# GloireLINVANI/3D_Gaussian_Splatting_Project

Measured on AMD Instinct MI355X. Metric: Gaussians·views/sec labelled (3M G, 1080p), majority vote; first vote_view submit -> labels on the host, higher is better.
Workload: dtype f64

## Files before the change

### 3d_gaussian_splatting_project_amd/csrc/gsx_ctx.hpp

```cpp
#pragma once
#include <hip/hip_runtime.h>

#include <chrono>
#include <cstdarg>
#include <cstdint>
#include <cstdio>
#include <map>
#include <cstddef>
#include <string>
#include <vector>

#include "../../include/gsx.h"
#include "host_pack.hpp"

namespace gsx {

void set_global_error(const char* fmt, ...);
struct Ctx;
int fail(Ctx* c, int code, const char* fmt, ...);

#define GSX_HIP(ctx, call)                                                                         \
    do {                                                                                           \
        hipError_t e__ = (call);                                                                   \
        if (e__ != hipSuccess)                                                                     \
// ... 224 lines not shown

    int64_t n = 0;
    int64_t n_pad = 0;
    DevBuf x, y, z;
    DevBuf perm;
    bool sorted = false;
    DevBuf sort_hist;

    int opt_spatial_sort = 1;
    int opt_xcd_swizzle = 32;
    int opt_vote_unroll = 8;
    int opt_slabs = 1;
    int opt_local_codes = 0;
    int opt_seg_tiled = 1;
    int opt_batched_counts = 1;
    int opt_seg_coarse = 1;
    int opt_flat_project = 1;

    bool vote_begun = false;
    int n_classes = 0, bins = 0;
    int first_view = 0, total_views = 0;
    bool wide = false;
    bool local_codes = false;
    int slabs = 1;
    int64_t sn = 0;
    std::vector<ViewDesc> views;
    DevBuf d_cull;
    int cull_pitch = 0;
    DevBuf d_cull_tally;
    int opt_wave_cull = 1;
    bool views_dirty = true;
    bool views_coarse = false;
    bool views_simple = false;
    DevBuf d_views;
    DevBuf segpool;
    size_t seg_used = 0;
    DevBuf errflag;
    HandOver ho;
    int opt_host_threads = 0;
    int opt_host_compact = 1;
#ifdef GSX_EXPERIMENTS
    int opt_ablate = 0;
#else
    static constexpr int opt_ablate = 0;
#endif
    int opt_labels_u8 = 1;
    int opt_host_pack = 1;
    void* h_labels = nullptr;
    size_t h_labels_cap = 0;
    hipEvent_t h_ev[kLabelChunks] = {nullptr, nullptr, nullptr, nullptr};
    void* h_views = nullptr;
    size_t h_views_cap = 0;
    hipEvent_t h_views_ev = nullptr;
    std::vector<ViewDesc> own_views;
    int own_first_view = 0;
    const void* pool_base = nullptr;
    int n_flushed = 0;
    bool planes_valid = false;
    bool planes_zero = false;
    bool planes_stale = false;
    DevBuf cnt, fv;
    DevBuf keys, labels;
    DevBuf labels8;
    DevBuf bcnt, bcodes;
    DevBuf cand, codes;
    long long counts_n = -1, counts_npad = -1, counts_sn = -1, codes_n = -1, codes_npad = -1;
    int counts_bins = -1;
    bool labels_valid = false;
    int opt_filter_project = 1;
    int opt_early_vote = 1;
    int opt_early_at = 0;
    std::chrono::steady_clock::time_point early_t0;
    int opt_early_replay = 1;
    bool early_replayed = false;
    int early_state = 0;
    int early_done = 0;
    int early_batches = 0;
    hipStream_t stream2 = nullptr;
    bool stream_borrowed = false;
    bool early_inflight = false;
    hipEvent_t early_maps_ev = nullptr, early_done_ev = nullptr, early_up_ev = nullptr;
    DevBuf ecnt, efv;
    DevBuf erec;
    DevBuf e_views, e_cull;
    void* h_early = nullptr;
    size_t h_early_cap = 0;

    RenderScene scene;
    RenderOpts ropt;
    RenderFrame frame;
    LiftState lift;
    Ctx* twins[kMaxFrames - 1] = {nullptr, nullptr, nullptr, nullptr, nullptr};
    DevBuf r_pre_args;
    std::vector<unsigned long long> r_pre_args_host;
    hipEvent_t r_pre_ev[kPreSets] = {nullptr, nullptr, nullptr};

    int opt_nn_brute = 0;
    DevBuf nn_index;
    int64_t nn_index_rows = 0;
    int nn_index_k = 0;
    DevBuf nn_pts, nn_cs;
    DevBuf nn_out, nn_flag;

    int opt_smooth_search = 0;
    DevBuf sm_lab[2];
    DevBuf sm_sup, sm_changed;
    DevBuf sm_lists;

    DevBuf sp_lab, sp_parent, sp_rep;
    DevBuf sp_size, sp_id, sp_kept;
    DevBuf sp_trip, sp_cnt;
    DevBuf sp_pts, sp_lists;

    int opt_iou_table_lds = 1;
    DevBuf iou_planes;
    DevBuf iou_cnt;
    DevBuf iou_ptrs;
    DevBuf iou_table;
    DevBuf iou_top;
    DevBuf iou_raw[2];
    void* iou_pin[2] = {nullptr, nullptr};
    size_t iou_pin_cap[2] = {0, 0};
    hipEvent_t iou_ev[2] = {nullptr, nullptr};
    bool iou_ev_pending[2] = {false, false};
    int iou_slot = 0;

    DevBuf seg_low;
    DevBuf q_bits;
    DevBuf q_parts;
    DevBuf q_tab;

    bool prof_on = false;
    std::vector<std::string> prof_names;
    std::vector<ProfEvent> prof_events;
    std::vector<hipEvent_t> event_pool;
    std::map<std::string, std::pair<int64_t, double>> prof_acc;
};

struct ProfScope {
    Ctx* c;
    ProfEvent ev{};
    bool active = false;
    hipStream_t st = nullptr;
    ProfScope(Ctx* ctx, const char* name, hipStream_t on = nullptr);
    ~ProfScope();
};

int vote_begin(Ctx* c, int n_classes, int first_view, int total_views);
int vote_view(Ctx* c, const gsx_camera* cam, const void* seg, int seg_dtype, int seg_w, int seg_h, int img_w, int img_h);
int early_pool_moves(Ctx* c);
void vote_release_host(Ctx* c);
int vote_slab_labels(Ctx* c, int slab, int slabs, int64_t* slab_size);
int vote_view_host(Ctx* c, const gsx_camera* cam, const void* seg, int seg_dtype, int seg_w, int seg_h, int img_w, int img_h);
int vote_views_device(Ctx* c, int n, const gsx_camera* cams, const void* const* segs, int seg_dtype, int seg_w, int seg_h,
                      int img_w, int img_h);
int vote_export(Ctx* c, int64_t reserve_bytes, void* blobs_out, void** pool_dev, int64_t* pool_bytes);
int vote_import(Ctx* c, int n_parts, const int32_t* part_views, const int64_t* part_offsets, const void* blobs,
                const void* pool_all_dev, int64_t pool_all_bytes);
int vote_import_uniform(Ctx* c, int n_parts, const int32_t* part_views, const int64_t* part_offsets, const gsx_camera* cams,
                        int seg_w, int seg_h, int img_w, int img_h, const void* pool_all_dev, int64_t pool_all_bytes);
int vote_import_undo(Ctx* c);
int vote_map_stride(Ctx* c, int seg_w, int seg_h, int64_t* stride);
int vote_views_match_uniform(Ctx* c, int n, const gsx_camera* cams, int seg_w, int seg_h, int img_w, int img_h, int32_t* match);
Workers* host_workers(Ctx* c, const void* near = nullptr);
int host_threads(Ctx* c);
int vote_flush_pending(Ctx* c);
void handover_release(Ctx* c);
// ... 124 lines not shown
```

### 3d_gaussian_splatting_project_amd/csrc/vote.hip

```cpp
#include <hip/hip_runtime.h>

#include <algorithm>
#include <chrono>
#include <cmath>
#include <cstring>
#include <type_traits>

#include "gsx_ctx.hpp"
#include "vote_device.hpp"

namespace gsx {

template <int DIV>
__global__ __launch_bounds__(kBlock) void project_kernel(const float* __restrict__ x, const float* __restrict__ y,
                                                         const float* __restrict__ z, long long n,
                                                         const ViewDesc* __restrict__ vd,
                                                         const uint32_t* __restrict__ perm, int* __restrict__ ox,
                                                         int* __restrict__ oy, float filt_h) {
    const long long i = (long long)blockIdx.x * kBlock + threadIdx.x;
    const bool valid = i < n;
    int xi, yi;
    const ViewRegs vr = load_view(vd);
    const double X = valid ? (double)x[i] : __builtin_nan(""), Y = valid ? (double)y[i] : 0.0, Z = valid ? (double)z[i] : 0.0;
    const bool vis = DIV == kDivFiltCoarse ? project_filtered(vr, filt_h, X, Y, Z, xi, yi) : project<DIV>(vr, X, Y, Z, xi, yi);
// ... 119 lines not shown
                                             double X, double Y, double Z, unsigned culled, int (&bin)[U], float filt_h) {
    if (DIV == kDivFlatCoarse || DIV == kDivFiltCoarse) {
        unsigned pixel[U];
#pragma unroll
        for (int u = 0; u < U; ++u) {
            const int v = vb - 1 - u;
            bin[u] = -1;
            if (((culled >> u) & 1u) || !(FULL || v >= 0)) continue;
            const ViewRegs vd = load_view(views + v);
            int xi, yi;
            if (DIV == kDivFiltCoarse ? project_filtered(vd, filt_h, X, Y, Z, xi, yi) : project<kDivFlatSimple>(vd, X, Y, Z, xi, yi)) {
                pixel[u] = (unsigned)xi | ((unsigned)yi << 16);
                const unsigned cx = (unsigned)xi >> 2, cy = (unsigned)yi >> 2;
                const unsigned coff = __umul24(cx >> 4, (unsigned)vd.coarse_row_bytes) + (cx & 15u) + (cy << 4);
                bin[u] = ((global_u8_ptr)((unsigned long long)vd.seg_off + vd.coarse_delta))[coff];
            }
        }
#pragma unroll
        for (int u = 0; u < U; ++u) {
            const bool mixed = bin[u] == 255;
            if (__builtin_amdgcn_ballot_w64(mixed) != 0) {
                const ViewDesc* __restrict__ vp = views + (vb - 1 - u);
                const global_u8_ptr base = (global_u8_ptr)(unsigned long long)vp->seg_off;
                const unsigned xi = pixel[u] & 0xffffu, yi = pixel[u] >> 16;
                if (mixed) bin[u] = base[__umul24(xi >> 4, (unsigned)vp->seg_row_bytes) + (xi & 15u) + (yi << 4)];
            }
        }
        return;
    }
#pragma unroll
    for (int u = 0; u < U; ++u) {
        const int v = vb - 1 - u;
        if ((culled >> u) & 1u) {
            bin[u] = -1;
            continue;
        }
        bin[u] = (FULL || v >= 0) ? seg_bin<DIV>(views + v, pool, X, Y, Z) : -1;
    }
}

template <int U, int DIV>
__global__ __launch_bounds__(kBlock) void vote_fused_labels_kernel(FusedParams p, const ViewDesc* __restrict__ views,
                                                                   int* __restrict__ labels) {
    extern __shared__ uint32_t lds[];
    uint32_t* row = lds + threadIdx.x * p.stride_dw;
    uint8_t* h = reinterpret_cast<uint8_t*>(row);

    for (int k = 0; k < p.stride_dw; ++k) row[k] = 0;
    const long long i = (long long)logical_block(blockIdx.x, gridDim.x, p.xcd_swizzle) * kBlock + threadIdx.x;
    const bool valid = i < p.n;
    const double X = valid ? (double)p.x[i] : __builtin_nan("");
    const double Y = valid ? (double)p.y[i] : 0.0;
    const double Z = valid ? (double)p.z[i] : 0.0;
    const uint8_t* __restrict__ pool = p.pool;

    int best = -1;
    int bestc = 0;
    const CullMasks cmask = wave_cull_masks(p.cull, p.cull_pitch, p.nviews, X, Y, Z, p.cull_tally);
    auto chunk = [&](auto full, int vb) {
        constexpr bool kFull = decltype(full)::value;
        int bin[U];
        gather_chunk<U, DIV, kFull>(views, pool, vb, X, Y, Z, cull_bits<U>(cmask, p.nviews - vb), bin, p.filt_h);
#pragma unroll
        for (int u = 0; u < U; ++u) {
            if (bin[u] >= 0) {
                const int c = h[bin[u]] + 1;
                h[bin[u]] = (uint8_t)c;
                if (c >= bestc) {
                    bestc = c;
                    best = bin[u];
                }
            }
        }
        };
    int vb = p.nviews;
    for (; vb >= U; vb -= U) chunk(std::true_type{}, vb);
    if (vb > 0) chunk(std::false_type{}, vb);
    if (valid) {
        const long long o = p.perm ? (long long)p.perm[i] : i;
        labels[o] = best - 1 + (best < 0);
    }
}

template <int U, int DIV>
__global__ __launch_bounds__(kBlock) void vote_record_kernel(FusedParams p, const ViewDesc* __restrict__ views,
                                                             uint8_t* __restrict__ rec) {
    const long long i = (long long)logical_block(blockIdx.x, gridDim.x, p.xcd_swizzle) * kBlock + threadIdx.x;
    const bool valid = i < p.n;
    const long long ic = valid ? i : 0;
    const float xf = p.x[ic], yf = p.y[ic], zf = p.z[ic];
    const double X = valid ? (double)xf : __builtin_nan("");
    const double Y = valid ? (double)yf : 0.0;
    const double Z = valid ? (double)zf : 0.0;
    const uint8_t* __restrict__ pool = p.pool;
    const int lane = threadIdx.x & 63;
    uint8_t* r = rec + (i - lane) * p.nviews + lane;
    const CullMasks cmask = wave_cull_masks(p.cull, p.cull_pitch, p.nviews, X, Y, Z, p.cull_tally);
    auto chunk = [&](auto full, int vb) {
        constexpr bool kFull = decltype(full)::value;
        int bin[U];
        gather_chunk<U, DIV, kFull>(views, pool, vb, X, Y, Z, cull_bits<U>(cmask, p.nviews - vb), bin, p.filt_h);
#pragma unroll
        for (int u = 0; u < U; ++u)
            if (kFull || vb - 1 - u >= 0) r[(vb - 1 - u) * 64] = (uint8_t)(bin[u] + 1);
    };
    int vb = p.nviews;
    for (; vb >= U; vb -= U) chunk(std::true_type{}, vb);
    if (vb > 0) chunk(std::false_type{}, vb);
}

template <int U, int DIV>
__global__ __launch_bounds__(kBlock) void vote_fused_replay_kernel(FusedParams p, const ViewDesc* __restrict__ views,
                                                                   const uint8_t* __restrict__ rec, int E,
                                                                   int* __restrict__ labels) {
    extern __shared__ uint32_t lds[];
    uint32_t* row = lds + threadIdx.x * p.stride_dw;
    uint8_t* h = reinterpret_cast<uint8_t*>(row);
    for (int k = 0; k < p.stride_dw; ++k) row[k] = 0;
    const long long i = (long long)logical_block(blockIdx.x, gridDim.x, p.xcd_swizzle) * kBlock + threadIdx.x;
    const bool valid = i < p.n;
    const long long ic = valid ? i : 0;
    const float xf = p.x[ic], yf = p.y[ic], zf = p.z[ic];
    const double X = valid ? (double)xf : __builtin_nan("");
    const double Y = valid ? (double)yf : 0.0;
    const double Z = valid ? (double)zf : 0.0;
    const uint8_t* __restrict__ pool = p.pool;
    int best = -1, bestc = 0;
    auto vote = [&](int b) {
        const int c = h[b] + 1;
        h[b] = (uint8_t)c;
        if (c >= bestc) {
            bestc = c;
            best = b;
        }
    };
    const CullMasks cmask = wave_cull_masks(p.cull, p.cull_pitch, p.nviews, X, Y, Z, p.cull_tally);
    auto chunk = [&](auto full, int vb) {
        constexpr bool kFull = decltype(full)::value;
        int bin[U];
        gather_chunk<U, DIV, kFull>(views, pool, vb, X, Y, Z, cull_bits<U>(cmask, p.nviews - vb), bin, p.filt_h);
#pragma unroll
        for (int u = 0; u < U; ++u)
            if (bin[u] >= 0) vote(bin[u]);
    };
    int vb = p.nviews;
    for (; vb >= U; vb -= U) chunk(std::true_type{}, vb);
    if (vb > 0) chunk(std::false_type{}, vb);
    constexpr int kReplay = 16;
    const int lane = threadIdx.x & 63;
    const uint8_t* __restrict__ r = rec + (i - lane) * E + lane;
    for (int v0 = E; v0 > 0; v0 -= kReplay) {
        unsigned b[kReplay];
#pragma unroll
        for (int j = 0; j < kReplay; ++j) {
            const int v = v0 - 1 - j;
            const unsigned got = r[max(v, 0) * 64];
            b[j] = v >= 0 ? got : 0u;
        }
#pragma unroll
        for (int j = 0; j < kReplay; ++j)
            if (b[j]) vote((int)b[j] - 1);
    }
    if (valid) {
        const long long o = p.perm ? (long long)p.perm[i] : i;
        labels[o] = best - 1 + (best < 0);
    }
}

typedef unsigned short u16x2 __attribute__((ext_vector_type(2)));
__device__ __forceinline__ uint32_t pk_max_u16(uint32_t a, uint32_t b) {
    return __builtin_bit_cast(uint32_t, __builtin_elementwise_max(__builtin_bit_cast(u16x2, a), __builtin_bit_cast(u16x2, b)));
}

template <int U, int DIV, int NQ>
__global__ __launch_bounds__(kBlock, 4) void vote_fused_final_kernel(FusedParams p, const ViewDesc* __restrict__ views,
                                                                     const uint8_t* __restrict__ cntA,
                                                                     const uint8_t* __restrict__ fvA,
                                                                     const uint8_t* __restrict__ recA, int E,
                                                                     int* __restrict__ labels, int ablate_arg) {
#ifdef GSX_EXPERIMENTS
    const int ablate = ablate_arg;
#else
    constexpr int ablate = 0;
#endif
    extern __shared__ uint32_t lds[];
    const long long i = (long long)logical_block(blockIdx.x, gridDim.x, p.xcd_swizzle) * kBlock + threadIdx.x;
    const bool valid = i < p.n;
    const long long ic = valid ? i : 0;
    const float xf = p.x[ic], yf = p.y[ic], zf = p.z[ic];
    const double X = valid ? (double)xf : __builtin_nan("");
    const double Y = valid ? (double)yf : 0.0;
    const double Z = valid ? (double)zf : 0.0;
    const uint8_t* __restrict__ pool = p.pool;
    const int lane = threadIdx.x & 63;
    const int g = lane >> 4;
    const int nq = (p.bins + 3) >> 2;
    uint32_t* wl = lds + (threadIdx.x >> 6) * (nq * 64);
    uint8_t* hw = reinterpret_cast<uint8_t*>(wl) + lane;
    const long long wave_at = (ablate & 1) ? 0 : (i - lane) * p.bins;
    const uint32_t* __restrict__ csrc = reinterpret_cast<const uint32_t*>(cntA + wave_at) + lane;
    const uint32_t* __restrict__ fsrc = reinterpret_cast<const uint32_t*>(fvA + wave_at) + lane;
    auto plane_dword = [&](const uint32_t* __restrict__ src, int q) {
        const uint32_t v = src[q * 64];
        return 4 * q + g < p.bins ? v : 0u;
    };
    constexpr int kRound = 13;
    uint32_t fd[NQ > 0 ? NQ : 1];
    if (NQ > 0) {
        uint32_t w[NQ > 0 ? NQ : 1];
#pragma unroll
        for (int q = 0; q < NQ; ++q) w[q] = plane_dword(csrc, q);
#pragma unroll
        for (int q = 0; q < NQ; ++q) fd[q] = plane_dword(fsrc, q);
        __builtin_amdgcn_sched_barrier(0);
#pragma unroll
        for (int q = 0; q < NQ; ++q)
            if (q < nq) wl[q * 64 + lane] = w[q];
    } else {
        for (int q0 = 0; q0 < nq; q0 += kRound) {
            uint32_t w[kRound];
#pragma unroll
            for (int j = 0; j < kRound; ++j) w[j] = plane_dword(csrc, q0 + j);
#pragma unroll
            for (int j = 0; j < kRound; ++j)
                if (q0 + j < nq) wl[(q0 + j) * 64 + lane] = w[j];
        }
    }
    __builtin_amdgcn_wave_barrier();

    int best = -1, bestc = 0;
    const CullMasks cmask = wave_cull_masks((ablate & 32) ? nullptr : p.cull, p.cull_pitch, p.nviews, X, Y, Z, p.cull_tally);
    auto chunk = [&](auto full, int vb) {
        constexpr bool kFull = decltype(full)::value;
        int bin[U];
        gather_chunk<U, DIV, kFull>(views, pool, vb, X, Y, Z, cull_bits<U>(cmask, p.nviews - vb), bin, p.filt_h);
#pragma unroll
        for (int u = 0; u < U; ++u) {
            if (bin[u] >= 0) {
                const int c = hw[bin[u] * 64] + 1;
                hw[bin[u] * 64] = (uint8_t)c;
                if (c >= bestc) {
                    bestc = c;
                    best = bin[u];
                }
// ... 654 lines not shown
    }
    return GSX_OK;
}

static int clear_stale_planes(Ctx* c) {
    if (!c->planes_stale) return GSX_OK;
    const size_t bytes = (size_t)c->bins * (size_t)c->n_pad * (c->wide ? 2 : 1);
    GSX_HIP(c, hipMemsetAsync(c->cnt.p, 0, bytes, c->stream));
    GSX_HIP(c, hipMemsetAsync(c->fv.p, 0, bytes, c->stream));
    c->planes_stale = false;
    c->planes_zero = true;
    return GSX_OK;
}

int vote_rewind(Ctx* c) {
    if (!c->vote_begun) return fail(c, GSX_E_STATE, "vote_rewind before vote_begin");
    GSX_HIP(c, hipSetDevice(c->device));
    c->n_flushed = 0;
    c->labels_valid = false;
    c->early_state = -1;
    c->early_batches = 0;
    if (const int rc = early_join(c)) return rc;
    if (c->planes_valid) {
        c->planes_valid = false;
        c->planes_zero = false;
        c->planes_stale = true;
    }
    return GSX_OK;
}

template <class K>
static int set_lds(Ctx* c, K kernel, size_t bytes) {
    if (bytes > 160 * 1024) return fail(c, GSX_E_UNSUPPORTED, "vote: %zu B of LDS per workgroup exceeds 160 KiB", bytes);
    GSX_HIP(c, hipFuncSetAttribute(reinterpret_cast<const void*>(kernel), hipFuncAttributeMaxDynamicSharedMemorySize,
                                   (int)bytes));
    return GSX_OK;
}

static constexpr int kUnroll = 8;

template <class K, class... Args>
static int launch_walk(Ctx* c, const char* name, hipStream_t st, K k, long long n, const FusedParams& p, Args... args) {
    const size_t lds = (size_t)kBlock * p.stride_dw * 4;
    const int rc = set_lds(c, k, lds);
    if (rc) return rc;
    ProfScope ps(c, name, st);
    hipLaunchKernelGGL(k, dim3(grid_for(n)), dim3(kBlock), lds, st, p, p.views, args...);
    GSX_HIP(c, hipGetLastError());
    return GSX_OK;
}
static inline size_t label_bytes(const Ctx* c) { return sizeof(int) * (size_t)(c->n_pad ? c->n_pad : 1); }

static constexpr int kEarlyPitch = 256;
static constexpr long long kEarlyMinGaussians = 1 << 18;
static constexpr int kEarlyMinViews = 32;
static constexpr double kEarlyUsPerGaussianView = 4.4e-6;
static constexpr double kRecordUsPerGaussianView = 1.7e-6;
static constexpr size_t kEarlySlack = 64 * 260;
static constexpr size_t kEarlyCullDoubles = (size_t)kCullStride * kCullPlanes * kEarlyPitch;

static bool early_common(const Ctx* c) {
    return c->opt_early_vote && c->first_view == 0 && !c->local_codes && c->slabs == 1 && c->n_flushed == 0 && !c->pool_base &&
           c->opt_flat_project && c->n > 0 && c->bins <= 255 &&
           (c->opt_early_vote == 2 || (c->n >= kEarlyMinGaussians && c->total_views >= kEarlyMinViews));
}
static bool early_possible(const Ctx* c) { return early_common(c) && c->total_views <= kMaxBatch && !c->wide; }
static bool early_batched_possible(const Ctx* c) { return early_common(c) && c->total_views > kMaxBatch && c->opt_batched_counts; }
static int early_batch_count(int total) {
    const int tail = std::min(std::max(total / 16, 16), 64), body = total - tail;
    return (body + kMaxBatch - 1) / kMaxBatch + 1;
}
static void early_batch_bounds(int total, int s, int& lo, int& hi) {
    const int tail = std::min(std::max(total / 16, 16), 64), body = total - tail;
    const int Sb = (body + kMaxBatch - 1) / kMaxBatch;
    if (s >= Sb) {
        lo = body;
        hi = total;
    } else {
        lo = (int)((long long)body * s / Sb);
        hi = (int)((long long)body * (s + 1) / Sb);
    }
}

static int early_upload(Ctx* c, int lo, int hi, int block, int blocks, hipStream_t st, int* dm) {
    const size_t vbytes = sizeof(ViewDesc) * kEarlyPitch, cbytes = sizeof(double) * kEarlyCullDoubles;
    if (!c->h_early) {
        GSX_HIP(c, hipHostMalloc(&c->h_early, vbytes + cbytes, hipHostMallocDefault));
        c->h_early_cap = vbytes + cbytes;
    }
    GSX_HIP(c, c->e_views.ensure(sizeof(ViewDesc) * (size_t)std::max(kEarlyPitch, c->total_views)));
    GSX_HIP(c, c->e_cull.ensure(cbytes * (size_t)std::max(2, blocks)));
    if (!c->early_up_ev) GSX_HIP(c, hipEventCreateWithFlags(&c->early_up_ev, hipEventDisableTiming));
    else GSX_HIP(c, hipEventSynchronize(c->early_up_ev));
    ViewDesc* hv = static_cast<ViewDesc*>(c->h_early);
    double* planes = reinterpret_cast<double*>(static_cast<char*>(c->h_early) + vbytes);
    std::memset(planes, 0, cbytes);
    const ViewKinds kinds = stage_views(c, lo, hi, c->segpool.p, hv, planes, kEarlyPitch);
    *dm = flat_div_mode(c, kinds.simple, kinds.coarse);
    if (hi > lo) GSX_HIP(c, hipMemcpyAsync(c->e_views.as<ViewDesc>() + lo, hv, sizeof(ViewDesc) * (size_t)(hi - lo), hipMemcpyHostToDevice, st));
    GSX_HIP(c, hipMemcpyAsync(c->e_cull.as<double>() + (size_t)block * kEarlyCullDoubles, planes, cbytes, hipMemcpyHostToDevice, st));
    GSX_HIP(c, hipEventRecord(c->early_up_ev, st));
    return GSX_OK;
}

static FusedParams early_params(Ctx* c, int lo, int hi, int block, int stride_bytes_per_bin) {
    FusedParams p = fused_params(c, stride_bytes_per_bin);
    p.views = c->e_views.as<ViewDesc>() + lo;
    p.nviews = hi - lo;
    p.cull = c->opt_wave_cull ? c->e_cull.as<double>() + (size_t)block * kEarlyCullDoubles : nullptr;
    p.cull_pitch = kEarlyPitch;
    return p;
}

int second_stream(Ctx* c) {
    if (c->stream2) return GSX_OK;
    int least = 0, greatest = 0;
    GSX_HIP(c, hipDeviceGetStreamPriorityRange(&least, &greatest));
    GSX_HIP(c, hipStreamCreateWithPriority(&c->stream2, hipStreamNonBlocking, least));
    return GSX_OK;
}

static int early_streams(Ctx* c) {
    const int rc = second_stream(c);
    if (rc) return rc;
    if (!c->early_maps_ev) GSX_HIP(c, hipEventCreateWithFlags(&c->early_maps_ev, hipEventDisableTiming));
    if (!c->early_done_ev) GSX_HIP(c, hipEventCreateWithFlags(&c->early_done_ev, hipEventDisableTiming));
    return GSX_OK;
}

int early_pool_moves(Ctx* c) {
    if (c->early_state == 1 || c->early_batches > 0) {
        GSX_HIP(c, hipStreamSynchronize(c->stream2));
        c->early_inflight = false;
        c->early_state = -1;
        c->early_batches = 0;
    }
    return GSX_OK;
}

static void early_release(Ctx* c) {
    if (c->stream2) {
        (void)hipStreamSynchronize(c->stream2);
        (void)hipStreamDestroy(c->stream2);
        c->stream2 = nullptr;
    }
    for (hipEvent_t* e : {&c->early_maps_ev, &c->early_done_ev, &c->early_up_ev}) {
        if (*e) (void)hipEventDestroy(*e);
        *e = nullptr;
    }
    if (c->h_early) (void)hipHostFree(c->h_early);
    c->h_early = nullptr;
    c->h_early_cap = 0;
    for (DevBuf* b : {&c->ecnt, &c->efv, &c->erec, &c->e_views, &c->e_cull}) b->release();
    c->early_state = -1;
}

static int early_batch_stage(Ctx* c) {
    const int nv = (int)c->views.size();
    const int S = early_batch_count(c->total_views);
    const int s = c->early_batches;
    if (s >= S - 1) return GSX_OK;
    int lo, hi;
    early_batch_bounds(c->total_views, s, lo, hi);
    if (nv != hi) return GSX_OK;
    int rc = vote_flush_pending(c);
    if (rc) return rc;
    if ((rc = early_streams(c))) return rc;
    const size_t plane = (size_t)c->bins * (size_t)c->n_pad;
    GSX_HIP(c, c->bcnt.ensure(plane * S));
    if ((rc = ensure_tally(c))) return rc;
    GSX_HIP(c, hipEventRecord(c->early_maps_ev, c->stream));
    GSX_HIP(c, hipStreamWaitEvent(c->stream2, c->early_maps_ev, 0));
    int dm = kDivFlat;
    if ((rc = early_upload(c, lo, hi, s, S, c->stream2, &dm))) return rc;
    const FusedParams p = early_params(c, lo, hi, s, 1);
    auto k = with_div<true>(dm, [](auto d) { return vote_fused_counts_kernel<kUnroll, decltype(d)::value>; });
    if ((rc = launch_walk(c, "vote_early_counts", c->stream2, k, c->n, p, c->bcnt.as<uint8_t>() + plane * s, (long long)c->n_pad))) return rc;
    GSX_HIP(c, hipEventRecord(c->early_done_ev, c->stream2));
    c->early_inflight = true;
    c->early_batches = s + 1;
    c->early_done = hi;
    return GSX_OK;
}

static int early_vote_stage(Ctx* c) {
    if (c->early_state == 0 && early_batched_possible(c)) return early_batch_stage(c);
    if (c->early_state != 0 || !early_possible(c)) return GSX_OK;
    const int nv = (int)c->views.size();
    int at;
    if (c->opt_early_at > 0) {
        at = std::max(1, (int)(((long long)c->total_views * c->opt_early_at + 999) / 1000));
        if (nv != at) return GSX_OK;
    } else {
        const auto now = std::chrono::steady_clock::now();
        if (nv == 1) c->early_t0 = now;
        if (nv < std::max(8, c->total_views / 4)) return GSX_OK;
        const double t_map = std::chrono::duration<double, std::micro>(now - c->early_t0).count() / (double)(nv - 1);
        const double t_view = (c->opt_early_replay ? kRecordUsPerGaussianView : kEarlyUsPerGaussianView) * (double)c->n;
        const int lo = (c->total_views + 1) / 2, hi = (int)(((long long)c->total_views * 880) / 1000);
        const int want = std::min(std::max((int)std::ceil(c->total_views * t_map / (t_map + t_view)), lo), std::max(lo, hi));
        if (nv < want) return GSX_OK;
        at = nv;
    }
    if (at >= c->total_views) return GSX_OK;
    int rc = vote_flush_pending(c);
    if (rc) return rc;
    if ((rc = early_streams(c))) return rc;
    const size_t plane = (size_t)c->bins * (size_t)c->n_pad;
    if (!c->opt_early_replay) {
        GSX_HIP(c, c->ecnt.ensure(plane + kEarlySlack));
        GSX_HIP(c, c->efv.ensure(plane + kEarlySlack));
    }
    GSX_HIP(c, c->erec.ensure((size_t)c->n_pad * (size_t)at));
    if ((rc = ensure_tally(c))) return rc;
    GSX_HIP(c, hipEventRecord(c->early_maps_ev, c->stream));
    GSX_HIP(c, hipStreamWaitEvent(c->stream2, c->early_maps_ev, 0));
    int dm = kDivFlat;
    if ((rc = early_upload(c, 0, at, 0, 2, c->stream2, &dm))) return rc;
    c->early_replayed = c->opt_early_replay != 0;
    if (c->early_replayed) {
        const FusedParams p = early_params(c, 0, at, 0, 1);
        auto kr = with_div<true>(dm, [](auto d) { return vote_record_kernel<kUnroll, decltype(d)::value>; });
        ProfScope ps(c, "vote_early_record", c->stream2);
        hipLaunchKernelGGL(kr, dim3(grid_for(c->n)), dim3(kBlock), 0, c->stream2, p, p.views, c->erec.as<uint8_t>());
        GSX_HIP(c, hipGetLastError());
    } else {
        const FusedParams p = early_params(c, 0, at, 0, 2);
        auto k = with_div<true>(dm, [](auto d) { return vote_fused_planes_kernel<kUnroll, uint8_t, decltype(d)::value>; });
        if ((rc = launch_walk(c, "vote_early_planes", c->stream2, k, c->n, p, c->ecnt.as<uint8_t>(), c->efv.as<uint8_t>(), 64LL, 0, 1, 0,
                              c->erec.as<uint8_t>())))
            return rc;
    }
    GSX_HIP(c, hipEventRecord(c->early_done_ev, c->stream2));
    c->early_inflight = true;
    c->early_done = at;
    c->early_state = 1;
    return GSX_OK;
}

int vote_view(Ctx* c, const gsx_camera* cam, const void* seg, int seg_dtype, int seg_w, int seg_h, int img_w, int img_h) {
    const int rc = vote_view_host(c, cam, seg, seg_dtype, seg_w, seg_h, img_w, img_h);
    return rc ? rc : early_vote_stage(c);
}

static int early_vote_finish(Ctx* c) {
    const int nv = (int)c->views.size();
    int rc = vote_flush_pending(c);
    if (rc) return rc;
    int dm = kDivFlat;
    if ((rc = early_upload(c, c->early_done, nv, 1, 2, c->stream, &dm))) return rc;
    GSX_HIP(c, c->labels.ensure(label_bytes(c)));
    if (c->early_replayed) {
        FusedParams pr = early_params(c, c->early_done, nv, 1, 1);
        auto kr = with_div<true>(dm, [](auto d) { return vote_fused_replay_kernel<kUnroll, decltype(d)::value>; });
        if ((rc = early_join(c))) return rc;
        if ((c->opt_ablate >> 4) & 2) pr.nviews = 0;
        return launch_walk(c, "vote_fused_replay", c->stream, kr, c->n, pr, c->erec.as<uint8_t>(), c->early_done, c->labels.as<int>());
    }
    FusedParams p = early_params(c, c->early_done, nv, 1, 1);
    const size_t lds = (size_t)(kBlock / 64) * ((c->bins + 3) / 4) * 256;
    constexpr int kRegRows = 38;
    const bool regs = c->bins <= 4 * kRegRows;
    auto k = with_div<true>(dm, [&](auto d) {
        constexpr int kDiv = decltype(d)::value;
        return regs ? vote_fused_final_kernel<kUnroll, kDiv, kRegRows> : vote_fused_final_kernel<kUnroll, kDiv, 0>;
    });
    if ((rc = set_lds(c, k, lds))) return rc;
    if ((rc = early_join(c))) return rc;
    const int ablate = (c->opt_ablate >> 4) & 63;
    if (ablate & 2) p.nviews = 0;
    ProfScope ps(c, "vote_fused_final");
    hipLaunchKernelGGL(k, dim3(grid_for(c->n)), dim3(kBlock), lds, c->stream, p, p.views, c->ecnt.as<uint8_t>(), c->efv.as<uint8_t>(),
                       c->erec.as<uint8_t>(), c->early_done, c->labels.as<int>(), ablate);
    GSX_HIP(c, hipGetLastError());
    return GSX_OK;
}

int vote_flush(Ctx* c) {
    if (!c->vote_begun) return fail(c, GSX_E_STATE, "vote_flush before vote_begin");
    GSX_HIP(c, hipSetDevice(c->device));
    int rc = early_join(c);
    if (rc) return rc;
    if ((rc = sync_views(c))) return rc;
    if ((rc = ensure_planes(c))) return rc;
    const int nv = (int)c->views.size();
    if (c->n <= 0 || c->n_flushed >= nv) {
        c->n_flushed = nv;
        return clear_stale_planes(c);
    }
    const FusedParams all = fused_params(c, 2);
    while (c->n_flushed < nv) {
        const int batch = std::min(kMaxBatch, nv - c->n_flushed);
        FusedParams p = all;
        p.views = all.views + c->n_flushed;
        p.nviews = batch;
        if (p.cull) p.cull = all.cull + c->n_flushed;
        const int view_base = c->first_view + c->n_flushed;
        const int fresh = (c->planes_zero || c->planes_stale) ? 1 : 0;
        auto planes = [&](auto t) {
            using PT = decltype(t);
            auto k = with_div(div_mode(c), [](auto d) { return vote_fused_planes_kernel<kUnroll, PT, decltype(d)::value>; });
            return launch_walk(c, "vote_fused_planes", c->stream, k, c->n, p, c->cnt.as<PT>(), c->fv.as<PT>(), (long long)c->sn, view_base,
                               fresh, c->local_codes ? 1 : 0, (uint8_t*)nullptr);
        };
        if ((rc = c->wide ? planes(uint16_t{}) : planes(uint8_t{}))) return rc;
        c->planes_zero = false;
        c->planes_stale = false;
        c->planes_valid = true;
        c->n_flushed += batch;
    }
    return GSX_OK;
}

int vote_tiebreak_keys(Ctx* c) {
    if (!c->vote_begun) return fail(c, GSX_E_STATE, "vote_tiebreak_keys before vote_begin");
    GSX_HIP(c, hipSetDevice(c->device));
    int rc = ensure_planes(c);
    if (rc) return rc;
    if ((rc = clear_stale_planes(c))) return rc;
    GSX_HIP(c, c->keys.ensure(label_bytes(c)));
    GSX_HIP(c, hipMemsetAsync(c->keys.p, 0, sizeof(int) * (size_t)c->n_pad, c->stream));
    if (c->n <= 0) return GSX_OK;
    ProfScope ps(c, "vote_keys");
    auto keys = [&](auto t) {
        using PT = decltype(t);
        hipLaunchKernelGGL(vote_keys_kernel<PT>, dim3(grid_for(c->n)), dim3(kBlock), 0, c->stream, c->cnt.as<PT>(), c->fv.as<PT>(),
                           (long long)c->n, (long long)c->sn, c->bins, c->keys.as<int>());
    };
    c->wide ? keys(uint16_t{}) : keys(uint8_t{});
    GSX_HIP(c, hipGetLastError());
    return GSX_OK;
}

static constexpr int kBadLabelWord = -2;
__global__ __launch_bounds__(kBlock) void labels_narrow_kernel(const int* __restrict__ labels, long long n, uint8_t* __restrict__ out,
                                                               int* __restrict__ errflag) {
    const long long i4 = ((long long)blockIdx.x * kBlock + threadIdx.x) * 4;
    if (i4 >= n) return;
    unsigned b[4];
    if (i4 + 4 <= n) {
// ... 355 lines not shown
```

Baseline: 97.14 billion.

## Pack early-vote records into 64-bit groups with per-wave skip masks

The early record kernel now stores bins for 8 views as one 64-bit word per lane, grouped per wave. It also writes a per-wave bitmask of which groups and views got any vote, so the replay kernel skips unvoted groups and reads packed words instead of single bytes. Separately, view descriptors and cull planes are merged into one staging buffer and uploaded with a single memcpy. This cuts record bandwidth and replay load count. The cost is extra bitmask logic, a 32-group (256-view) limit on the early stage, and an occupancy hint on the record kernel.

```diff
diff --git a/3d_gaussian_splatting_project_amd/csrc/gsx_ctx.hpp b/3d_gaussian_splatting_project_amd/csrc/gsx_ctx.hpp
--- a/3d_gaussian_splatting_project_amd/csrc/gsx_ctx.hpp
+++ b/3d_gaussian_splatting_project_amd/csrc/gsx_ctx.hpp
@@ -330,7 +330,8 @@
     hipEvent_t early_maps_ev = nullptr, early_done_ev = nullptr, early_up_ev = nullptr;
     DevBuf ecnt, efv;
     DevBuf erec;
-    DevBuf e_views, e_cull;
+    DevBuf emask;
+    DevBuf e_stage;
     void* h_early = nullptr;
     size_t h_early_cap = 0;
 
diff --git a/3d_gaussian_splatting_project_amd/csrc/vote.hip b/3d_gaussian_splatting_project_amd/csrc/vote.hip
--- a/3d_gaussian_splatting_project_amd/csrc/vote.hip
+++ b/3d_gaussian_splatting_project_amd/csrc/vote.hip
@@ -225,9 +225,26 @@
     }
 }
 
-template <int U, int DIV>
-__global__ __launch_bounds__(kBlock) void vote_record_kernel(FusedParams p, const ViewDesc* __restrict__ views,
-                                                             uint8_t* __restrict__ rec) {
+static constexpr int kRecGroup = 8;
+static constexpr int kMaskWords = 4;
+static inline size_t record_bytes(long long n_pad, int E) {
+    return (size_t)(n_pad / 64) * (size_t)((E + kRecGroup - 1) / kRecGroup) * 64 * sizeof(unsigned long long);
+}
+static inline size_t record_mask_bytes(long long n_pad) { return (size_t)(n_pad / 64) * kMaskWords * sizeof(unsigned long long); }
+
+__device__ __forceinline__ unsigned cull_bits_at(const CullMasks& k, int done) {
+    auto word = [&](int w) { return w == 0 ? k.m[0] : w == 1 ? k.m[1] : w == 2 ? k.m[2] : w == 3 ? k.m[3] : 0ull; };
+    const int d = done + 64, w = (d >> 6) - 1, sh = d & 63;
+    unsigned long long bits = word(w) >> sh;
+    if (sh) bits |= word(w + 1) << (64 - sh);
+    unsigned out = (unsigned)bits & 0xffu;
+    if (done < 0) out |= (1u << -done) - 1u;
+    return out;
+}
+
+template <int DIV>
+__global__ __launch_bounds__(kBlock) __attribute__((amdgpu_waves_per_eu(8))) void vote_record_kernel(
+    FusedParams p, const ViewDesc* __restrict__ views, unsigned long long* __restrict__ rec, unsigned long long* __restrict__ rowmask) {
     const long long i = (long long)logical_block(blockIdx.x, gridDim.x, p.xcd_swizzle) * kBlock + threadIdx.x;
     const bool valid = i < p.n;
     const long long ic = valid ? i : 0;
@@ -237,24 +254,49 @@
     const double Z = valid ? (double)zf : 0.0;
     const uint8_t* __restrict__ pool = p.pool;
     const int lane = threadIdx.x & 63;
-    uint8_t* r = rec + (i - lane) * p.nviews + lane;
+    const int G = (p.nviews + kRecGroup - 1) / kRecGroup;
+    const long long wave = i >> 6;
+    unsigned long long* r = rec + wave * G * 64 + lane;
     const CullMasks cmask = wave_cull_masks(p.cull, p.cull_pitch, p.nviews, X, Y, Z, p.cull_tally);
-    auto chunk = [&](auto full, int vb) {
-        constexpr bool kFull = decltype(full)::value;
-        int bin[U];
-        gather_chunk<U, DIV, kFull>(views, pool, vb, X, Y, Z, cull_bits<U>(cmask, p.nviews - vb), bin, p.filt_h);
-#pragma unroll
-        for (int u = 0; u < U; ++u)
-            if (kFull || vb - 1 - u >= 0) r[(vb - 1 - u) * 64] = (uint8_t)(bin[u] + 1);
-    };
-    int vb = p.nviews;
-    for (; vb >= U; vb -= U) chunk(std::true_type{}, vb);
-    if (vb > 0) chunk(std::false_type{}, vb);
+    unsigned long long m0 = 0, m1 = 0, m2 = 0, m3 = 0;
+    for (int w = (G - 1) >> 3; w >= 0; --w) {
+        unsigned long long acc = 0;
+        for (int g = min(G, 8 * w + 8) - 1; g >= 8 * w; --g) {
+            const ViewDesc* __restrict__ gv = views + kRecGroup * g;
+            const int done = p.nviews - kRecGroup * (g + 1);
+            int bin[kRecGroup];
+            gather_chunk<kRecGroup, DIV, true>(gv, pool, kRecGroup, X, Y, Z, cull_bits_at(cmask, done), bin, p.filt_h);
+            unsigned lo = 0, hi = 0, voted = 0;
+#pragma unroll
+            for (int u = 0; u < kRecGroup; ++u) {
+                const int k = kRecGroup - 1 - u;
+                const unsigned b = (unsigned)(bin[u] + 1);
+                if (k < 4) lo |= b << (8 * k);
+                else hi |= b << (8 * (k - 4));
+                if (__builtin_amdgcn_ballot_w64(bin[u] >= 0) != 0) voted |= 1u << k;
+            }
+            if (voted) {
+                r[g * 64] = (unsigned long long)lo | ((unsigned long long)hi << 32);
+                acc |= (unsigned long long)voted << (8 * (g & 7));
+            }
+        }
+        m0 = w == 0 ? acc : m0;
+        m1 = w == 1 ? acc : m1;
+        m2 = w == 2 ? acc : m2;
+        m3 = w == 3 ? acc : m3;
+    }
+    if (lane < kMaskWords) rowmask[wave * kMaskWords + lane] = lane == 0 ? m0 : lane == 1 ? m1 : lane == 2 ? m2 : m3;
+}
+
+__device__ __forceinline__ unsigned long long uniform_u64(unsigned long long v) {
+    const unsigned lo = __builtin_amdgcn_readfirstlane((unsigned)v), hi = __builtin_amdgcn_readfirstlane((unsigned)(v >> 32));
+    return (unsigned long long)lo | ((unsigned long long)hi << 32);
 }
 
 template <int U, int DIV>
 __global__ __launch_bounds__(kBlock) void vote_fused_replay_kernel(FusedParams p, const ViewDesc* __restrict__ views,
-                                                                   const uint8_t* __restrict__ rec, int E,
+                                                                   const unsigned long long* __restrict__ rec,
+                                                                   const unsigned long long* __restrict__ rowmask, int E,
                                                                    int* __restrict__ labels) {
     extern __shared__ uint32_t lds[];
     uint32_t* row = lds + threadIdx.x * p.stride_dw;
@@ -289,20 +331,37 @@
     int vb = p.nviews;
     for (; vb >= U; vb -= U) chunk(std::true_type{}, vb);
     if (vb > 0) chunk(std::false_type{}, vb);
-    constexpr int kReplay = 16;
     const int lane = threadIdx.x & 63;
-    const uint8_t* __restrict__ r = rec + (i - lane) * E + lane;
-    for (int v0 = E; v0 > 0; v0 -= kReplay) {
-        unsigned b[kReplay];
-#pragma unroll
-        for (int j = 0; j < kReplay; ++j) {
-            const int v = v0 - 1 - j;
-            const unsigned got = r[max(v, 0) * 64];
-            b[j] = v >= 0 ? got : 0u;
-        }
-#pragma unroll
-        for (int j = 0; j < kReplay; ++j)
-            if (b[j]) vote((int)b[j] - 1);
+    const long long wave = __builtin_amdgcn_readfirstlane((int)(i >> 6));
+    const unsigned long long* __restrict__ mk = rowmask + wave * kMaskWords;
+    const unsigned long long mk0 = uniform_u64(mk[0]), mk1 = uniform_u64(mk[1]), mk2 = uniform_u64(mk[2]), mk3 = uniform_u64(mk[3]);
+    const int G = (E + kRecGroup - 1) / kRecGroup;
+    const unsigned long long* __restrict__ r = rec + wave * G * 64 + lane;
+    for (int k = (G - 1) >> 3; k >= 0; --k) {
+        const unsigned long long m = k == 0 ? mk0 : k == 1 ? mk1 : k == 2 ? mk2 : mk3;
+        if (m == 0) continue;
+        const unsigned mh[2] = {(unsigned)m, (unsigned)(m >> 32)};
+        unsigned lo[8], hi[8];
+#pragma unroll
+        for (int j = 0; j < 8; ++j) {
+            lo[j] = hi[j] = 0;
+            if ((mh[j >> 2] >> (8 * (j & 3))) & 0xffu) {
+                const unsigned long long w = r[(8 * k + j) * 64];
+                lo[j] = (unsigned)w;
+                hi[j] = (unsigned)(w >> 32);
+            }
+        }
+#pragma unroll
+        for (int j = 7; j >= 0; --j) {
+            if (((mh[j >> 2] >> (8 * (j & 3))) & 0xffu) == 0) continue;
+#pragma unroll
+            for (int b = 7; b >= 0; --b) {
+                if ((mh[j >> 2] >> (8 * (j & 3) + b)) & 1u) {
+                    const unsigned bin = ((b < 4 ? lo[j] : hi[j]) >> (8 * (b & 3))) & 0xffu;
+                    if (bin) vote((int)bin - 1);
+                }
+            }
+        }
     }
     if (valid) {
         const long long o = p.perm ? (long long)p.perm[i] : i;
@@ -1123,32 +1182,36 @@
     }
 }
 
+static constexpr size_t kEarlyCullBytes = sizeof(double) * kEarlyCullDoubles;
+static constexpr size_t kEarlyBlockBytes = kEarlyCullBytes + sizeof(ViewDesc) * kEarlyPitch;
+static_assert(kEarlyCullBytes % 64 == 0, "the descriptors behind the planes keep their alignment");
+
 static int early_upload(Ctx* c, int lo, int hi, int block, int blocks, hipStream_t st, int* dm) {
-    const size_t vbytes = sizeof(ViewDesc) * kEarlyPitch, cbytes = sizeof(double) * kEarlyCullDoubles;
+    if (hi - lo > kEarlyPitch) return fail(c, GSX_E_STATE, "early_upload: %d views in one stage", hi - lo);
     if (!c->h_early) {
-        GSX_HIP(c, hipHostMalloc(&c->h_early, vbytes + cbytes, hipHostMallocDefault));
-        c->h_early_cap = vbytes + cbytes;
-    }
-    GSX_HIP(c, c->e_views.ensure(sizeof(ViewDesc) * (size_t)std::max(kEarlyPitch, c->total_views)));
-    GSX_HIP(c, c->e_cull.ensure(cbytes * (size_t)std::max(2, blocks)));
+        GSX_HIP(c, hipHostMalloc(&c->h_early, kEarlyBlockBytes, hipHostMallocDefault));
+        c->h_early_cap = kEarlyBlockBytes;
+    }
+    GSX_HIP(c, c->e_stage.ensure(kEarlyBlockBytes * (size_t)std::max(2, blocks)));
     if (!c->early_up_ev) GSX_HIP(c, hipEventCreateWithFlags(&c->early_up_ev, hipEventDisableTiming));
     else GSX_HIP(c, hipEventSynchronize(c->early_up_ev));
-    ViewDesc* hv = static_cast<ViewDesc*>(c->h_early);
-    double* planes = reinterpret_cast<double*>(static_cast<char*>(c->h_early) + vbytes);
-    std::memset(planes, 0, cbytes);
+    double* planes = static_cast<double*>(c->h_early);
+    ViewDesc* hv = reinterpret_cast<ViewDesc*>(static_cast<char*>(c->h_early) + kEarlyCullBytes);
+    std::memset(planes, 0, kEarlyCullBytes);
     const ViewKinds kinds = stage_views(c, lo, hi, c->segpool.p, hv, planes, kEarlyPitch);
     *dm = flat_div_mode(c, kinds.simple, kinds.coarse);
-    if (hi > lo) GSX_HIP(c, hipMemcpyAsync(c->e_views.as<ViewDesc>() + lo, hv, sizeof(ViewDesc) * (size_t)(hi - lo), hipMemcpyHostToDevice, st));
-    GSX_HIP(c, hipMemcpyAsync(c->e_cull.as<double>() + (size_t)block * kEarlyCullDoubles, planes, cbytes, hipMemcpyHostToDevice, st));
+    GSX_HIP(c, hipMemcpyAsync(c->e_stage.as<char>() + (size_t)block * kEarlyBlockBytes, c->h_early,
+                              kEarlyCullBytes + sizeof(ViewDesc) * (size_t)std::max(hi - lo, 0), hipMemcpyHostToDevice, st));
     GSX_HIP(c, hipEventRecord(c->early_up_ev, st));
     return GSX_OK;
 }
 
 static FusedParams early_params(Ctx* c, int lo, int hi, int block, int stride_bytes_per_bin) {
     FusedParams p = fused_params(c, stride_bytes_per_bin);
-    p.views = c->e_views.as<ViewDesc>() + lo;
+    char* at = c->e_stage.as<char>() + (size_t)block * kEarlyBlockBytes;
+    p.views = reinterpret_cast<const ViewDesc*>(at + kEarlyCullBytes);
     p.nviews = hi - lo;
-    p.cull = c->opt_wave_cull ? c->e_cull.as<double>() + (size_t)block * kEarlyCullDoubles : nullptr;
+    p.cull = c->opt_wave_cull ? reinterpret_cast<const double*>(at) : nullptr;
     p.cull_pitch = kEarlyPitch;
     return p;
 }
@@ -1192,7 +1255,7 @@
     if (c->h_early) (void)hipHostFree(c->h_early);
     c->h_early = nullptr;
     c->h_early_cap = 0;
-    for (DevBuf* b : {&c->ecnt, &c->efv, &c->erec, &c->e_views, &c->e_cull}) b->release();
+    for (DevBuf* b : {&c->ecnt, &c->efv, &c->erec, &c->emask, &c->e_stage}) b->release();
     c->early_state = -1;
 }
 
@@ -1252,7 +1315,12 @@
         GSX_HIP(c, c->ecnt.ensure(plane + kEarlySlack));
         GSX_HIP(c, c->efv.ensure(plane + kEarlySlack));
     }
-    GSX_HIP(c, c->erec.ensure((size_t)c->n_pad * (size_t)at));
+    if (c->opt_early_replay) {
+        GSX_HIP(c, c->erec.ensure(record_bytes(c->n_pad, at)));
+        GSX_HIP(c, c->emask.ensure(record_mask_bytes(c->n_pad)));
+    } else {
+        GSX_HIP(c, c->erec.ensure((size_t)c->n_pad * (size_t)at));
+    }
     if ((rc = ensure_tally(c))) return rc;
     GSX_HIP(c, hipEventRecord(c->early_maps_ev, c->stream));
     GSX_HIP(c, hipStreamWaitEvent(c->stream2, c->early_maps_ev, 0));
@@ -1261,9 +1329,10 @@
     c->early_replayed = c->opt_early_replay != 0;
     if (c->early_replayed) {
         const FusedParams p = early_params(c, 0, at, 0, 1);
-        auto kr = with_div<true>(dm, [](auto d) { return vote_record_kernel<kUnroll, decltype(d)::value>; });
+        auto kr = with_div<true>(dm, [](auto d) { return vote_record_kernel<decltype(d)::value>; });
         ProfScope ps(c, "vote_early_record", c->stream2);
-        hipLaunchKernelGGL(kr, dim3(grid_for(c->n)), dim3(kBlock), 0, c->stream2, p, p.views, c->erec.as<uint8_t>());
+        hipLaunchKernelGGL(kr, dim3(grid_for(c->n)), dim3(kBlock), 0, c->stream2, p, p.views, c->erec.as<unsigned long long>(),
+                           c->emask.as<unsigned long long>());
         GSX_HIP(c, hipGetLastError());
     } else {
         const FusedParams p = early_params(c, 0, at, 0, 2);
@@ -1296,7 +1365,8 @@
         auto kr = with_div<true>(dm, [](auto d) { return vote_fused_replay_kernel<kUnroll, decltype(d)::value>; });
         if ((rc = early_join(c))) return rc;
         if ((c->opt_ablate >> 4) & 2) pr.nviews = 0;
-        return launch_walk(c, "vote_fused_replay", c->stream, kr, c->n, pr, c->erec.as<uint8_t>(), c->early_done, c->labels.as<int>());
+        return launch_walk(c, "vote_fused_replay", c->stream, kr, c->n, pr, (const unsigned long long*)c->erec.as<unsigned long long>(),
+                           (const unsigned long long*)c->emask.as<unsigned long long>(), c->early_done, c->labels.as<int>());
     }
     FusedParams p = early_params(c, c->early_done, nv, 1, 1);
     const size_t lds = (size_t)(kBlock / 64) * ((c->bins + 3) / 4) * 256;
```

New measurement: 93.57 billion. -3.7%, worse.
